# chengstone/cchess-zero

Hardware: AMD Instinct MI355X
Metric: MCTS simulations/sec (whole node), playout=1600, 7-block net (higher is better)
Workload: dtype mx6

## Files before the change

### cchess_zero_amd/csrc/cz_trunk_mx.h

```cpp
#pragma once
#include "cz_conv_kernel.h"

namespace czconv {

#include "cz_trunk_mx_asm.inc"

struct MXGeo {
    static constexpr int P = 2;
    static constexpr int ROWS = P * 90;
    static constexpr int THREADS = 512;
    static constexpr int ENT = 224;
    static constexpr int XPLANE = ENT * 16, YPLANE = ENT * 8, SPLANE = ENT * 4;
    static constexpr int X_OFF = 0, Y_OFF = 8 * XPLANE, S_OFF = Y_OFF + 8 * YPLANE;
    static constexpr int HI_OFF = S_OFF + 2 * SPLANE;
    static constexpr int ZERO_OFF = HI_OFF + ROWS * CV_ROWB;
    static constexpr int W_OFF = ZERO_OFF + CV_ROWB;
    static constexpr int SLAB_BYTES = 16384;
    static constexpr int SLAB_SHIFT = 14;
    static constexpr int SLABS_PER_LAYER = 36;
    static constexpr int LDS_BYTES = W_OFF + TW_NBUF * SLAB_BYTES;
    static constexpr int PLANES_OFF = W_OFF + 3 * SLAB_BYTES;
    static constexpr int HEADW_OFF = LDS_BYTES;
    static constexpr int LDS_TOTAL = LDS_BYTES + 3 * 128 * 4;
    static constexpr int F32_ROWB = 512;
};
static_assert(MXGeo::HI_OFF % 256 == 0 && MXGeo::W_OFF % 16 == 0, "hi rows are swizzled by their absolute 256-byte row");
static_assert(MXGeo::Y_OFF == 28672 && MXGeo::S_OFF == 43008, "tools/gen_tower_asm.py: MX_Y_OFF / MX_S_OFF");
static_assert(MXGeo::ROWS * MXGeo::F32_ROWB <= MXGeo::HEADW_OFF, "fp32 trunk rows must leave the head weights alone");
constexpr int MX_P = MXGeo::P, MX_THREADS = MXGeo::THREADS, MX_LDS_BYTES = MXGeo::LDS_TOTAL;

typedef unsigned u32x6 __attribute__((ext_vector_type(6)));
typedef _Float16 f16x8 __attribute__((ext_vector_type(8)));

__device__ __forceinline__ u32x6 mx_cvt6(f32x16 a, f32x16 b, float scale) {
    u32x6 r;
    asm volatile("v_cvt_scalef32_2xpk16_fp6_f32 %0, %1, %2, %3" : "=&v"(r) : "v"(a), "v"(b), "v"(scale));
    return r;
}

__global__ __launch_bounds__(512, 2) void k_trunk_mx_c128(const unsigned char *__restrict__ wpk,
                                                           const float *__restrict__ bias,
                                                           float *__restrict__ out,
                                                           const float *__restrict__ head_w,
                                                           const float *__restrict__ head_b,
                                                           float *__restrict__ head_out,
                                                           const uint16_t *__restrict__ planes,
                                                           const uint16_t *__restrict__ w0,
                                                           const float *__restrict__ b0,
                                                           int B, int nlayers,
                                                           const int *__restrict__ bcount,
                                                           unsigned long long *__restrict__ clk) {
    extern __shared__ __attribute__((aligned(16))) unsigned char smem[];
    using Geo = MXGeo;
    const int tid = threadIdx.x, lane = tid & 63, wave = tid >> 6;
    const int wr = wave >> 2, ct = wave & 3;
    const int l31 = lane & 31, khalf = lane >> 5;
    const int pos0 = blockIdx.x * Geo::P;
    if (bcount) {
        const int live = *bcount;
        B = live < B ? live : B;
    }
    if (pos0 >= B) return;
    unsigned long long clk_c0 = 0, clk_r0 = 0;
    if (clk) { clk_c0 = __builtin_readcyclecounter(); clk_r0 = __builtin_amdgcn_s_memrealtime(); }
    const int npos = (B - pos0) < Geo::P ? (B - pos0) : Geo::P;
    const int nrows = npos * 90;
    const int nslabs = nlayers * Geo::SLABS_PER_LAYER;
    auto lds_addr = [](int row_byte_off, int c) { return row_byte_off + ((c ^ ((row_byte_off >> 8) & 15)) << 4); };
    const unsigned voff0 = (unsigned)tid << 4, voff1 = voff0 + (unsigned)Geo::THREADS * 16u;
    const int wave_u = __builtin_amdgcn_readfirstlane(wave);
    auto lds_row_of = [](int natural) {
        const int p = natural / 90, c = natural - p * 90, y = c / 10, x = c - y * 10;
        return 20 * y + 10 * p + x;
    };

    trunk_ring_prologue<Geo>(smem, wpk, nslabs, wave_u, voff0, voff1);
    trunk_stage_planes<Geo>(smem, planes, pos0, nrows, tid);
    if (tid < 16) *reinterpret_cast<uint4 *>(smem + Geo::ZERO_OFF + (tid << 4)) = make_uint4(0, 0, 0, 0);
    if (tid < 256) *reinterpret_cast<uint4 *>(smem + Geo::X_OFF + (tid >> 5) * Geo::XPLANE + (192 + (tid & 31)) * 16) = make_uint4(0, 0, 0, 0);
    else *reinterpret_cast<uint2 *>(smem + Geo::Y_OFF + ((tid - 256) >> 5) * Geo::YPLANE + (192 + (tid & 31)) * 8) = make_uint2(0, 0);
    if (tid < 64) *reinterpret_cast<uint32_t *>(smem + Geo::S_OFF + (tid >> 5) * Geo::SPLANE + (192 + (tid & 31)) * 4) = 0x7f7f7f7fu;
    if (head_out && tid < 3 * 128 / 4)
        reinterpret_cast<float4 *>(smem + Geo::HEADW_OFF)[tid] = reinterpret_cast<const float4 *>(head_w)[tid];
    bf16x8 wf[9][2];
#pragma unroll
    for (int t = 0; t < 9; ++t)
#pragma unroll
        for (int part = 0; part < 2; ++part)
            wf[t][part] = *reinterpret_cast<const bf16x8 *>(w0 + ((size_t)(((t * 2 + part) * 2 + khalf) * 128 + ct * 32 + l31) << 3));
    asm volatile("s_waitcnt vmcnt(0)" ::: "memory");
    __syncthreads();

    int rowk[3], tapmask[3], natb[3];
#pragma unroll
    for (int i = 0; i < 3; ++i) {
        const int k = 32 * (wr * 3 + i) + l31 - 12;
        const int kk = k < 0 ? 0 : k;
        const int h = kk / 20, rem = kk - h * 20, pp = rem / 10, w = rem - pp * 10;
        rowk[i] = k;
        natb[i] = (pp * 90 + h * 10 + w) * 32;
        int m = 0;
        for (int t = 0; t < 9; ++t) {
            const int y = h + t / 3 - 1, x = w + t % 3 - 1;
            if (k >= 0 && y >= 0 && y < 9 && x >= 0 && x < 10) m |= 1 << t;
        }
        tapmask[i] = m;
    }
    auto tap_addr = [&](int tap, int (&ab)[3], int (&key)[3], int (&xr)[3], int (&yr)[3]) {
        const int delta = (tap / 3 - 1) * 20 + (tap - (tap / 3) * 3 - 1);
#pragma unroll
        for (int i = 0; i < 3; ++i) {
            const int kk = rowk[i] + delta;
            const bool on = (tapmask[i] >> tap) & 1;
            const int rb = Geo::HI_OFF + kk * CV_ROWB;
            ab[i] = on ? rb : Geo::ZERO_OFF;
            key[i] = ((rb >> 8) & 15) ^ khalf;
            xr[i] = khalf * Geo::XPLANE + ((on ? kk : 192 + (kk & 31)) << 4);
            yr[i] = xr[i] >> 1;
        }
    };
    const int vb0 = Geo::W_OFF + khalf * 2048 + ((ct * 32 + l31) << 4);
    const int vy0 = Geo::W_OFF + 12288 + khalf * 1024 + ((ct * 32 + l31) << 3);
    const int vs0 = Geo::W_OFF + 14336 + khalf * 512 + ((ct * 32 + l31) << 2);
    int keep;

    int rkk[3];
    auto refresh_rk = [&]() {
#pragma unroll
        for (int i = 0; i < 3; ++i) {
            rkk[i] = rowk[i] < 0 ? 0 : rowk[i];
            asm volatile("" : "+v"(rkk[i]));
        }
    };
    f32x16 xreg[3];
    float4 bqn[4];
    auto load_bias = [&](const float *bl) {
        int t = threadIdx.x;
        asm volatile("" : "+v"(t));
        const int boff = ((t >> 6) & 3) * 32 + 4 * ((t & 63) >> 5);
#pragma unroll
        for (int q = 0; q < 4; ++q) bqn[q] = *reinterpret_cast<const float4 *>(bl + boff + 8 * q);
    };
    auto init_acc = [&](f32x16 (&acc)[3], const float *bl, bool add_x) {
#pragma unroll
        for (int q = 0; q < 4; ++q) {
            const float4 bq = bl ? *reinterpret_cast<const float4 *>(bl + ct * 32 + 8 * q + 4 * khalf) : bqn[q];
#pragma unroll
            for (int i = 0; i < 3; ++i) {
                acc[i][4 * q + 0] = bq.x + (add_x ? xreg[i][4 * q + 0] : 0.0f);
                acc[i][4 * q + 1] = bq.y + (add_x ? xreg[i][4 * q + 1] : 0.0f);
                acc[i][4 * q + 2] = bq.z + (add_x ? xreg[i][4 * q + 2] : 0.0f);
                acc[i][4 * q + 3] = bq.w + (add_x ? xreg[i][4 * q + 3] : 0.0f);
            }
        }
    };
    auto store_tile = [&](f32x16 a, int i, bool keep_x) {
        f32x16 v;
#pragma unroll
        for (int r = 0; r < 16; ++r) v[r] = __builtin_amdgcn_fmed3f(a[r], 0.0f, 65504.0f);
        if (keep_x) xreg[i] = v;
        uint32_t pk[8];
        f32x16 hi, lo;
#pragma unroll
        for (int r = 0; r < 16; r += 2) {
            pk[r >> 1] = pack_pair<true>(f32x2{v[r], v[r + 1]});
            const f32x2 u = unpack_pair<true>(pk[r >> 1]);
            hi[r] = u[0]; hi[r + 1] = u[1];
            lo[r] = (v[r] - u[0]) * 2048.0f; lo[r + 1] = (v[r + 1] - u[1]) * 2048.0f;
        }
        float m = v[0];
#pragma unroll
        for (int r = 1; r < 16; ++r) m = fmaxf(m, v[r]);
        int byte = (int)(__float_as_uint(m) >> 23) - 2;
        byte = byte < 1 ? 1 : byte;
        const u32x6 blk = mx_cvt6(hi, lo, __uint_as_float((uint32_t)byte << 23));
        const bool live = rowk[i] >= 0;
        if (live) {
            const int rowb = Geo::HI_OFF + rkk[i] * CV_ROWB;
#pragma unroll
            for (int q = 0; q < 4; ++q) {
                const int n0 = ct * 32 + 8 * q + 4 * khalf;
                *reinterpret_cast<uint2 *>(smem + lds_addr(rowb, n0 >> 3) + ((n0 & 4) << 1)) = make_uint2(pk[2 * q], pk[2 * q + 1]);
            }
            const int g = 2 * ct + khalf;
            *reinterpret_cast<uint4 *>(smem + Geo::X_OFF + g * Geo::XPLANE + (rkk[i] << 4)) = make_uint4(blk[0], blk[1], blk[2], blk[3]);
            *reinterpret_cast<uint2 *>(smem + Geo::Y_OFF + g * Geo::YPLANE + (rkk[i] << 3)) = make_uint2(blk[4], blk[5]);
            smem[Geo::S_OFF + khalf * Geo::SPLANE + (rkk[i] << 2) + ct] = (unsigned char)byte;
        }
    };
    auto store_tile_f32 = [&](f32x16 a, int i) {
        if (rowk[i] < 0) return;
#pragma unroll
        for (int q = 0; q < 4; ++q) {
            const int c = 8 * ct + 2 * q + khalf;
            *reinterpret_cast<float4 *>(smem + rkk[i] * Geo::F32_ROWB + ((c ^ (rkk[i] & 31)) << 4)) =
                make_float4(fmaxf(a[4 * q + 0], 0.0f), fmaxf(a[4 * q + 1], 0.0f), fmaxf(a[4 * q + 2], 0.0f), fmaxf(a[4 * q + 3], 0.0f));
        }
    };

    {
        f32x16 acc[3];
        init_acc(acc, b0, false);
        load_bias(bias);
#pragma unroll
        for (int t = 0; t < 9; ++t) {
            const int shift = (t / 3 - 1) * 10 + (t % 3 - 1);
            bf16x8 af[3];
#pragma unroll
            for (int i = 0; i < 3; ++i) {
                const int a = ((tapmask[i] >> t) & 1) ? Geo::PLANES_OFF + (natb[i] + shift * 32) : Geo::ZERO_OFF;
                af[i] = *reinterpret_cast<const bf16x8 *>(smem + a + khalf * 16);
            }
#pragma unroll
            for (int part = 0; part < 2; ++part)
#pragma unroll
                for (int i = 0; i < 3; ++i)
                    acc[i] = mfma_32x32x16<true>(wf[t][part], af[i], acc[i]);
        }
        refresh_rk();
#pragma unroll
        for (int i = 0; i < 3; ++i) store_tile(acc[i], i, true);
        __syncthreads();
    }

#define MX_OPERANDS(NAB, NKEY)                                                                                       \
            : [c0] "+v"(acc[0]), [c1] "+v"(acc[1]), [c2] "+v"(acc[2]),                                                 \
              [a0h0] "+v"(fa.a[0]), [a0h1] "+v"(fa.a[1]), [a0h2] "+v"(fa.a[2]), [w0] "+v"(fa.w),                      \
              [a1h0] "+v"(fb.a[0]), [a1h1] "+v"(fb.a[1]), [a1h2] "+v"(fb.a[2]), [w1] "+v"(fb.w),                      \
              [sb0] "+v"(sb[0]), [sb1] "+v"(sb[1]), [sb2] "+v"(sb[2]),                                                \
              [t0] "=&v"(t0), [t1] "=&v"(t1), [t2] "=&v"(t2), [ws] "=&v"(wsr), [keep] "=&s"(keep)                      \
            : [ab0] "v"(ab[0]), [ab1] "v"(ab[1]), [ab2] "v"(ab[2]), [key0] "v"(key[0]), [key1] "v"(key[1]),            \
              [key2] "v"(key[2]), [nab0] "v"(NAB[0]), [nab1] "v"(NAB[1]), [nab2] "v"(NAB[2]), [nkey0] "v"(NKEY[0]),     \
              [nkey1] "v"(NKEY[1]), [nkey2] "v"(NKEY[2]), [xr0] "v"(xr[0]), [xr1] "v"(xr[1]), [xr2] "v"(xr[2]),        \
              [yr0] "v"(yr[0]), [yr1] "v"(yr[1]), [yr2] "v"(yr[2]), [vb] "v"(vb), [vy] "v"(vy), [vs] "v"(vs),          \
              [vbn] "v"(vbn), [voff0] "v"(voff0), [voff1] "v"(voff1), [sbase] "s"(sbase), [ldst] "s"(ldst)
#define MX_CLOBBERS "memory", "scc", "v232", "v233", "v234", "v235", "v236", "v237", "v238", "v239", "v240", "v241", "v242", "v243", \
                    "v244", "v245", "v246", "v247", "v248", "v249", "v250", "v251", "v252", "v253", "v254", "v255"
#define MX_ARGS()                                                                                                    \
            TRUNK_SLAB_ARGS(wpk, const int vy = vy0 + slot; const int vs = vs0 + slot;)
#define MX_RUN(ASMSTR, NAB, NKEY)                                                                                    \
        {                                                                                                            \
            MX_ARGS()                                                                                                \
            asm volatile(ASMSTR MX_OPERANDS(NAB, NKEY) : MX_CLOBBERS);                                               \
            ++g;                                                                                                     \
        }
#define MX_RUNV(ASMSTR, NAB, NKEY)                           \
        {                                                                                                            \
            MX_ARGS()                                                                                                \
            asm volatile(ASMSTR MX_OPERANDS(NAB, NKEY), [skipm] "s"(skipm) : MX_CLOBBERS, "vcc");                    \
            ++g;                                                                                                     \
        }

#ifdef MX_TIMING
    unsigned long long tm_loop = 0, tm_epi = 0, tm_set = 0, tm_t0 = __builtin_readcyclecounter();
    const unsigned long long tm_first = tm_t0 - clk_c0;
#define MX_TM(acc) { const unsigned long long n_ = __builtin_readcyclecounter(); acc += n_ - tm_t0; tm_t0 = n_; }
#else
#define MX_TM(acc)
#endif
    struct MxFrag { bf16x8 a[3], w; };
    int g = 0;
    int skipm;
    asm volatile("s_cmp_lt_u32 %1, 4\n\ts_cselect_b32 %0, 1, 0" : "=s"(skipm) : "s"(wave_u) : "scc");
#pragma unroll 1
    for (int layer = 0; layer < nlayers; ++layer) {
        f32x16 acc[3];
        init_acc(acc, nullptr, (layer & 1) != 0);
        int ab[3], key[3], nab[3], nkey[3], xr[3], yr[3], nxr[3], nyr[3], t0, t1, t2, wsr;
        int sb[3] = {0, 0, 0};
        MxFrag fa, fb;
        tap_addr(0, ab, key, xr, yr);
        {
            const int vb = vb0 + (((unsigned)g & 3u) << Geo::SLAB_SHIFT);
#pragma unroll
            for (int i = 0; i < 3; ++i) {
                fa.a[i] = *reinterpret_cast<const bf16x8 *>(smem + ab[i] + ((0 ^ key[i]) << 4));
                fb.a[i] = *reinterpret_cast<const bf16x8 *>(smem + ab[i] + ((2 ^ key[i]) << 4));
            }
            fa.w = *reinterpret_cast<const bf16x8 *>(smem + vb);
            fb.w = *reinterpret_cast<const bf16x8 *>(smem + vb + 4096);
            asm volatile("" : "+v"(fa.a[0]), "+v"(fa.a[1]), "+v"(fa.a[2]), "+v"(fa.w), "+v"(fb.a[0]), "+v"(fb.a[1]), "+v"(fb.a[2]), "+v"(fb.w));
        }
        MX_TM(tm_set)
        int tap = 0;
#pragma unroll 1
        for (; tap < 3; ++tap) {
            MX_RUNV(MX_SKIP0_ASM_Q0, ab, key)
            MX_RUNV(MX_SKIP0_ASM_Q1, ab, key)
            MX_RUNV(MX_SKIP0_ASM_Q2, ab, key)
            tap_addr(tap + 1, nab, nkey, nxr, nyr);
            MX_RUNV(MX_SKIP0_ASM_Q3, nab, nkey)
#pragma unroll
            for (int i = 0; i < 3; ++i) { ab[i] = nab[i]; key[i] = nkey[i]; xr[i] = nxr[i]; yr[i] = nyr[i]; }
        }
#pragma unroll 1
        for (; tap < 8; ++tap) {
            MX_RUN(MX_SLAB_ASM_Q0, ab, key)
            MX_RUN(MX_SLAB_ASM_Q1, ab, key)
            MX_RUN(MX_SLAB_ASM_Q2, ab, key)
            tap_addr(tap + 1, nab, nkey, nxr, nyr);
            MX_RUN(MX_SLAB_ASM_Q3, nab, nkey)
#pragma unroll
            for (int i = 0; i < 3; ++i) { ab[i] = nab[i]; key[i] = nkey[i]; xr[i] = nxr[i]; yr[i] = nyr[i]; }
        }
        MX_RUN(MX_SLAB_ASM_Q0, ab, key)
        MX_RUN(MX_SLAB_ASM_Q1, ab, key)
        MX_RUN(MX_SLAB_ASM_Q2, ab, key)
        MX_RUN(MX_SLAB_ASM_Q3_LAST, ab, key)
        const bool last = layer + 1 == nlayers;
        if (last) asm volatile("s_waitcnt vmcnt(0)" ::: "memory");
        else load_bias(bias + (layer + 1) * 128);
        asm volatile("s_nop 15\n\ts_nop 15\n\ts_nop 15" ::: "memory");
        MX_TM(tm_loop)
        refresh_rk();
        if (last) {
#pragma unroll
            for (int i = 0; i < 3; ++i) store_tile_f32(acc[i], i);
        } else {
#pragma unroll
            for (int i = 0; i < 3; ++i) store_tile(acc[i], i, (layer & 1) != 0);
        }
        __syncthreads();
        MX_TM(tm_epi)
    }
    if (clk && tid == 0) {
        clk[blockIdx.x * 4 + 0] = clk_c0; clk[blockIdx.x * 4 + 1] = __builtin_readcyclecounter();
        clk[blockIdx.x * 4 + 2] = clk_r0; clk[blockIdx.x * 4 + 3] = __builtin_amdgcn_s_memrealtime();
#ifdef MX_TIMING
        clk[blockIdx.x * 4 + 0] = tm_first; clk[blockIdx.x * 4 + 1] = tm_loop; clk[blockIdx.x * 4 + 2] = tm_epi; clk[blockIdx.x * 4 + 3] = tm_set;
#endif
    }
    asm volatile("s_waitcnt vmcnt(0)" ::: "memory");
    if (out) {
        float4 *go = reinterpret_cast<float4 *>(out + (size_t)pos0 * 90 * 128);
        for (int idx = tid; idx < nrows * 32; idx += Geo::THREADS) {
            const int r = idx >> 5, c = idx & 31, k = lds_row_of(r);
            go[idx] = *reinterpret_cast<const float4 *>(smem + k * Geo::F32_ROWB + ((c ^ (k & 31)) << 4));
        }
    }
    if (head_out) {
        const float *hw = reinterpret_cast<const float *>(smem + Geo::HEADW_OFF);
        for (int r = tid; r < nrows; r += Geo::THREADS) {
            const int k = lds_row_of(r);
            float acc0 = 0.f, acc1 = 0.f, acc2 = 0.f;
#pragma unroll 4
            for (int c = 0; c < 32; ++c) {
                const float4 e = *reinterpret_cast<const float4 *>(smem + k * Geo::F32_ROWB + ((c ^ (k & 31)) << 4));
                const float *w0_ = hw + c * 4, *w1_ = hw + 128 + c * 4, *w2_ = hw + 256 + c * 4;
                acc0 += e.x * w0_[0] + e.y * w0_[1] + e.z * w0_[2] + e.w * w0_[3];
                acc1 += e.x * w1_[0] + e.y * w1_[1] + e.z * w1_[2] + e.w * w1_[3];
                acc2 += e.x * w2_[0] + e.y * w2_[1] + e.z * w2_[2] + e.w * w2_[3];
            }
            float *o = head_out + ((size_t)pos0 * 90 + r) * 3;
            o[0] = fmaxf(acc0 + head_b[0], 0.f);
            o[1] = fmaxf(acc1 + head_b[1], 0.f);
            o[2] = fmaxf(acc2 + head_b[2], 0.f);
        }
    }
}
#undef MX_OPERANDS
#undef MX_CLOBBERS
#undef MX_ARGS
#undef MX_RUN
#undef MX_RUNV

}
```

### cchess_zero_amd/csrc/cz_trunk_mx_asm.inc

```
#define MX_SLAB_ASM_Q0 \
    "s_mov_b32 %[keep], m0\n\t" \
    "s_waitcnt lgkmcnt(4)\n\t" \
    "v_mfma_f32_32x32x16_f16 %[c0], %[w0], %[a0h0], %[c0]\n\t" \
    "ds_read_b128 v[232:235], %[xr0] offset:0\n\t" \
    "ds_read_b64 v[236:237], %[yr0] offset:28672\n\t" \
    "ds_read_b128 v[238:241], %[xr1] offset:0\n\t" \
    "ds_read_b64 v[242:243], %[yr1] offset:28672\n\t" \
    "v_lshrrev_b32 %[t0], 1, %[yr0]\n\t" \
    "v_lshrrev_b32 %[t1], 1, %[yr1]\n\t" \
    "v_lshrrev_b32 %[t2], 1, %[yr2]\n\t" \
    "v_mfma_f32_32x32x16_f16 %[c1], %[w0], %[a0h1], %[c1]\n\t" \
    "ds_read_b128 v[244:247], %[xr2] offset:0\n\t" \
    "ds_read_b64 v[248:249], %[yr2] offset:28672\n\t" \
    "ds_read_b32 %[sb0], %[t0] offset:43008\n\t" \
    "ds_read_b32 %[sb1], %[t1] offset:43008\n\t" \
    "ds_read_b32 %[sb2], %[t2] offset:43008\n\t" \
    "v_mfma_f32_32x32x16_f16 %[c2], %[w0], %[a0h2], %[c2]\n\t" \
    "ds_read_b128 v[250:253], %[vb] offset:8192\n\t" \
    "ds_read_b64 v[254:255], %[vy]\n\t" \
    "ds_read_b32 %[ws], %[vs]\n\t" \
    "s_waitcnt vmcnt(2)\n\t" \
    "s_barrier\n\t" \
    "s_waitcnt lgkmcnt(12)\n\t" \
    "v_mfma_f32_32x32x16_f16 %[c0], %[w1], %[a1h0], %[c0]\n\t" \
    "v_xor_b32 %[t0], 4, %[key0]\n\t" \
    "v_xor_b32 %[t1], 4, %[key1]\n\t" \
    "v_xor_b32 %[t2], 4, %[key2]\n\t" \
    "v_lshl_add_u32 %[t0], %[t0], 4, %[ab0]\n\t" \
    "v_lshl_add_u32 %[t1], %[t1], 4, %[ab1]\n\t" \
    "v_lshl_add_u32 %[t2], %[t2], 4, %[ab2]\n\t" \
    "v_mfma_f32_32x32x16_f16 %[c1], %[w1], %[a1h1], %[c1]\n\t" \
    "ds_read_b128 %[a0h0], %[t0]\n\t" \
    "ds_read_b128 %[a0h1], %[t1]\n\t" \
    "v_mfma_f32_32x32x16_f16 %[c2], %[w1], %[a1h2], %[c2]\n\t" \
    "ds_read_b128 %[a0h2], %[t2]\n\t" \
    "ds_read_b128 %[w0], %[vbn]\n\t" \
    "s_waitcnt lgkmcnt(4)\n\t" \
    "v_mfma_scale_f32_32x32x64_f8f6f4 %[c0], v[250:255], v[232:237], %[c0], %[ws], %[sb0] op_sel:[0,0,0] op_sel_hi:[0,0,0] cbsz:2 blgp:2\n\t" \
    "v_xor_b32 %[t0], 6, %[key0]\n\t" \
    "v_xor_b32 %[t1], 6, %[key1]\n\t" \
    "v_xor_b32 %[t2], 6, %[key2]\n\t" \
    "v_lshl_add_u32 %[t0], %[t0], 4, %[ab0]\n\t" \
    "v_lshl_add_u32 %[t1], %[t1], 4, %[ab1]\n\t" \
    "v_lshl_add_u32 %[t2], %[t2], 4, %[ab2]\n\t" \
    "s_mov_b32 m0, %[ldst]\n\t" \
    "s_nop 0\n\t" \
    "global_load_lds_dwordx4 %[voff0], %[sbase]\n\t" \
    "v_mfma_scale_f32_32x32x64_f8f6f4 %[c1], v[250:255], v[238:243], %[c1], %[ws], %[sb1] op_sel:[0,0,0] op_sel_hi:[0,0,0] cbsz:2 blgp:2\n\t" \
    "ds_read_b128 %[a1h0], %[t0]\n\t" \
    "ds_read_b128 %[a1h1], %[t1]\n\t" \
    "s_add_u32 m0, %[ldst], 0x2000\n\t" \
    "s_nop 0\n\t" \
    "global_load_lds_dwordx4 %[voff1], %[sbase]\n\t" \
    "v_mfma_scale_f32_32x32x64_f8f6f4 %[c2], v[250:255], v[244:249], %[c2], %[ws], %[sb2] op_sel:[0,0,0] op_sel_hi:[0,0,0] cbsz:2 blgp:2\n\t" \
    "ds_read_b128 %[a1h2], %[t2]\n\t" \
    "ds_read_b128 %[w1], %[vbn] offset:4096\n\t" \
    "s_mov_b32 m0, %[keep]\n\t"

#define MX_SLAB_ASM_Q1 \
    "s_mov_b32 %[keep], m0\n\t" \
    "s_waitcnt lgkmcnt(4)\n\t" \
    "v_mfma_f32_32x32x16_f16 %[c0], %[w0], %[a0h0], %[c0]\n\t" \
    "ds_read_b128 v[232:235], %[xr0] offset:7168\n\t" \
    "ds_read_b64 v[236:237], %[yr0] offset:32256\n\t" \
    "ds_read_b128 v[238:241], %[xr1] offset:7168\n\t" \
    "ds_read_b64 v[242:243], %[yr1] offset:32256\n\t" \
    "v_mfma_f32_32x32x16_f16 %[c1], %[w0], %[a0h1], %[c1]\n\t" \
    "ds_read_b128 v[244:247], %[xr2] offset:7168\n\t" \
    "ds_read_b64 v[248:249], %[yr2] offset:32256\n\t" \
    "v_mfma_f32_32x32x16_f16 %[c2], %[w0], %[a0h2], %[c2]\n\t" \
    "ds_read_b128 v[250:253], %[vb] offset:8192\n\t" \
    "ds_read_b64 v[254:255], %[vy]\n\t" \
    "ds_read_b32 %[ws], %[vs]\n\t" \
    "s_waitcnt vmcnt(2)\n\t" \
    "s_barrier\n\t" \
    "s_waitcnt lgkmcnt(9)\n\t" \
    "v_mfma_f32_32x32x16_f16 %[c0], %[w1], %[a1h0], %[c0]\n\t" \
    "v_xor_b32 %[t0], 8, %[key0]\n\t" \
    "v_xor_b32 %[t1], 8, %[key1]\n\t" \
    "v_xor_b32 %[t2], 8, %[key2]\n\t" \
    "v_lshl_add_u32 %[t0], %[t0], 4, %[ab0]\n\t" \
    "v_lshl_add_u32 %[t1], %[t1], 4, %[ab1]\n\t" \
    "v_lshl_add_u32 %[t2], %[t2], 4, %[ab2]\n\t" \
    "v_mfma_f32_32x32x16_f16 %[c1], %[w1], %[a1h1], %[c1]\n\t" \
    "ds_read_b128 %[a0h0], %[t0]\n\t" \
    "ds_read_b128 %[a0h1], %[t1]\n\t" \
    "v_mfma_f32_32x32x16_f16 %[c2], %[w1], %[a1h2], %[c2]\n\t" \
    "ds_read_b128 %[a0h2], %[t2]\n\t" \
    "ds_read_b128 %[w0], %[vbn]\n\t" \
    "s_waitcnt lgkmcnt(4)\n\t" \
    "v_mfma_scale_f32_32x32x64_f8f6f4 %[c0], v[250:255], v[232:237], %[c0], %[ws], %[sb0] op_sel:[0,1,0] op_sel_hi:[0,0,0] cbsz:2 blgp:2\n\t" \
    "v_xor_b32 %[t0], 10, %[key0]\n\t" \
    "v_xor_b32 %[t1], 10, %[key1]\n\t" \
    "v_xor_b32 %[t2], 10, %[key2]\n\t" \
    "v_lshl_add_u32 %[t0], %[t0], 4, %[ab0]\n\t" \
    "v_lshl_add_u32 %[t1], %[t1], 4, %[ab1]\n\t" \
    "v_lshl_add_u32 %[t2], %[t2], 4, %[ab2]\n\t" \
    "s_mov_b32 m0, %[ldst]\n\t" \
    "s_nop 0\n\t" \
    "global_load_lds_dwordx4 %[voff0], %[sbase]\n\t" \
    "v_mfma_scale_f32_32x32x64_f8f6f4 %[c1], v[250:255], v[238:243], %[c1], %[ws], %[sb1] op_sel:[0,1,0] op_sel_hi:[0,0,0] cbsz:2 blgp:2\n\t" \
    "ds_read_b128 %[a1h0], %[t0]\n\t" \
    "ds_read_b128 %[a1h1], %[t1]\n\t" \
    "s_add_u32 m0, %[ldst], 0x2000\n\t" \
    "s_nop 0\n\t" \
    "global_load_lds_dwordx4 %[voff1], %[sbase]\n\t" \
    "v_mfma_scale_f32_32x32x64_f8f6f4 %[c2], v[250:255], v[244:249], %[c2], %[ws], %[sb2] op_sel:[0,1,0] op_sel_hi:[0,0,0] cbsz:2 blgp:2\n\t" \
    "ds_read_b128 %[a1h2], %[t2]\n\t" \
    "ds_read_b128 %[w1], %[vbn] offset:4096\n\t" \
    "s_mov_b32 m0, %[keep]\n\t"

#define MX_SLAB_ASM_Q2 \
    "s_mov_b32 %[keep], m0\n\t" \
    "s_waitcnt lgkmcnt(4)\n\t" \
    "v_mfma_f32_32x32x16_f16 %[c0], %[w0], %[a0h0], %[c0]\n\t" \
    "ds_read_b128 v[232:235], %[xr0] offset:14336\n\t" \
    "ds_read_b64 v[236:237], %[yr0] offset:35840\n\t" \
    "ds_read_b128 v[238:241], %[xr1] offset:14336\n\t" \
    "ds_read_b64 v[242:243], %[yr1] offset:35840\n\t" \
    "v_mfma_f32_32x32x16_f16 %[c1], %[w0], %[a0h1], %[c1]\n\t" \
    "ds_read_b128 v[244:247], %[xr2] offset:14336\n\t" \
    "ds_read_b64 v[248:249], %[yr2] offset:35840\n\t" \
    "v_mfma_f32_32x32x16_f16 %[c2], %[w0], %[a0h2], %[c2]\n\t" \
    "ds_read_b128 v[250:253], %[vb] offset:8192\n\t" \
    "ds_read_b64 v[254:255], %[vy]\n\t" \
    "ds_read_b32 %[ws], %[vs]\n\t" \
    "s_waitcnt vmcnt(2)\n\t" \
    "s_barrier\n\t" \
    "s_waitcnt lgkmcnt(9)\n\t" \
    "v_mfma_f32_32x32x16_f16 %[c0], %[w1], %[a1h0], %[c0]\n\t" \
    "v_xor_b32 %[t0], 12, %[key0]\n\t" \
    "v_xor_b32 %[t1], 12, %[key1]\n\t" \
    "v_xor_b32 %[t2], 12, %[key2]\n\t" \
    "v_lshl_add_u32 %[t0], %[t0], 4, %[ab0]\n\t" \
    "v_lshl_add_u32 %[t1], %[t1], 4, %[ab1]\n\t" \
    "v_lshl_add_u32 %[t2], %[t2], 4, %[ab2]\n\t" \
    "v_mfma_f32_32x32x16_f16 %[c1], %[w1], %[a1h1], %[c1]\n\t" \
    "ds_read_b128 %[a0h0], %[t0]\n\t" \
    "ds_read_b128 %[a0h1], %[t1]\n\t" \
    "v_mfma_f32_32x32x16_f16 %[c2], %[w1], %[a1h2], %[c2]\n\t" \
    "ds_read_b128 %[a0h2], %[t2]\n\t" \
    "ds_read_b128 %[w0], %[vbn]\n\t" \
    "s_waitcnt lgkmcnt(4)\n\t" \
    "v_mfma_scale_f32_32x32x64_f8f6f4 %[c0], v[250:255], v[232:237], %[c0], %[ws], %[sb0] op_sel:[0,0,0] op_sel_hi:[0,1,0] cbsz:2 blgp:2\n\t" \
    "v_xor_b32 %[t0], 14, %[key0]\n\t" \
    "v_xor_b32 %[t1], 14, %[key1]\n\t" \
    "v_xor_b32 %[t2], 14, %[key2]\n\t" \
    "v_lshl_add_u32 %[t0], %[t0], 4, %[ab0]\n\t" \
    "v_lshl_add_u32 %[t1], %[t1], 4, %[ab1]\n\t" \
    "v_lshl_add_u32 %[t2], %[t2], 4, %[ab2]\n\t" \
    "s_mov_b32 m0, %[ldst]\n\t" \
    "s_nop 0\n\t" \
    "global_load_lds_dwordx4 %[voff0], %[sbase]\n\t" \
    "v_mfma_scale_f32_32x32x64_f8f6f4 %[c1], v[250:255], v[238:243], %[c1], %[ws], %[sb1] op_sel:[0,0,0] op_sel_hi:[0,1,0] cbsz:2 blgp:2\n\t" \
    "ds_read_b128 %[a1h0], %[t0]\n\t" \
    "ds_read_b128 %[a1h1], %[t1]\n\t" \
    "s_add_u32 m0, %[ldst], 0x2000\n\t" \
    "s_nop 0\n\t" \
    "global_load_lds_dwordx4 %[voff1], %[sbase]\n\t" \
    "v_mfma_scale_f32_32x32x64_f8f6f4 %[c2], v[250:255], v[244:249], %[c2], %[ws], %[sb2] op_sel:[0,0,0] op_sel_hi:[0,1,0] cbsz:2 blgp:2\n\t" \
    "ds_read_b128 %[a1h2], %[t2]\n\t" \
    "ds_read_b128 %[w1], %[vbn] offset:4096\n\t" \
    "s_mov_b32 m0, %[keep]\n\t"

#define MX_SLAB_ASM_Q3 \
    "s_mov_b32 %[keep], m0\n\t" \
    "s_waitcnt lgkmcnt(4)\n\t" \
    "v_mfma_f32_32x32x16_f16 %[c0], %[w0], %[a0h0], %[c0]\n\t" \
    "ds_read_b128 v[232:235], %[xr0] offset:21504\n\t" \
    "ds_read_b64 v[236:237], %[yr0] offset:39424\n\t" \
    "ds_read_b128 v[238:241], %[xr1] offset:21504\n\t" \
    "ds_read_b64 v[242:243], %[yr1] offset:39424\n\t" \
    "v_mfma_f32_32x32x16_f16 %[c1], %[w0], %[a0h1], %[c1]\n\t" \
    "ds_read_b128 v[244:247], %[xr2] offset:21504\n\t" \
    "ds_read_b64 v[248:249], %[yr2] offset:39424\n\t" \
    "v_mfma_f32_32x32x16_f16 %[c2], %[w0], %[a0h2], %[c2]\n\t" \
    "ds_read_b128 v[250:253], %[vb] offset:8192\n\t" \
    "ds_read_b64 v[254:255], %[vy]\n\t" \
    "ds_read_b32 %[ws], %[vs]\n\t" \
    "s_waitcnt vmcnt(2)\n\t" \
    "s_barrier\n\t" \
    "s_waitcnt lgkmcnt(9)\n\t" \
    "v_mfma_f32_32x32x16_f16 %[c0], %[w1], %[a1h0], %[c0]\n\t" \
    "v_xor_b32 %[t0], 0, %[nkey0]\n\t" \
    "v_xor_b32 %[t1], 0, %[nkey1]\n\t" \
    "v_xor_b32 %[t2], 0, %[nkey2]\n\t" \
    "v_lshl_add_u32 %[t0], %[t0], 4, %[nab0]\n\t" \
    "v_lshl_add_u32 %[t1], %[t1], 4, %[nab1]\n\t" \
    "v_lshl_add_u32 %[t2], %[t2], 4, %[nab2]\n\t" \
    "v_mfma_f32_32x32x16_f16 %[c1], %[w1], %[a1h1], %[c1]\n\t" \
    "ds_read_b128 %[a0h0], %[t0]\n\t" \
    "ds_read_b128 %[a0h1], %[t1]\n\t" \
    "v_mfma_f32_32x32x16_f16 %[c2], %[w1], %[a1h2], %[c2]\n\t" \
    "ds_read_b128 %[a0h2], %[t2]\n\t" \
    "ds_read_b128 %[w0], %[vbn]\n\t" \
    "s_waitcnt lgkmcnt(4)\n\t" \
    "v_mfma_scale_f32_32x32x64_f8f6f4 %[c0], v[250:255], v[232:237], %[c0], %[ws], %[sb0] op_sel:[0,1,0] op_sel_hi:[0,1,0] cbsz:2 blgp:2\n\t" \
    "v_xor_b32 %[t0], 2, %[nkey0]\n\t" \
    "v_xor_b32 %[t1], 2, %[nkey1]\n\t" \
    "v_xor_b32 %[t2], 2, %[nkey2]\n\t" \
    "v_lshl_add_u32 %[t0], %[t0], 4, %[nab0]\n\t" \
    "v_lshl_add_u32 %[t1], %[t1], 4, %[nab1]\n\t" \
    "v_lshl_add_u32 %[t2], %[t2], 4, %[nab2]\n\t" \
    "s_mov_b32 m0, %[ldst]\n\t" \
    "s_nop 0\n\t" \
    "global_load_lds_dwordx4 %[voff0], %[sbase]\n\t" \
    "v_mfma_scale_f32_32x32x64_f8f6f4 %[c1], v[250:255], v[238:243], %[c1], %[ws], %[sb1] op_sel:[0,1,0] op_sel_hi:[0,1,0] cbsz:2 blgp:2\n\t" \
    "ds_read_b128 %[a1h0], %[t0]\n\t" \
    "ds_read_b128 %[a1h1], %[t1]\n\t" \
    "s_add_u32 m0, %[ldst], 0x2000\n\t" \
    "s_nop 0\n\t" \
    "global_load_lds_dwordx4 %[voff1], %[sbase]\n\t" \
    "v_mfma_scale_f32_32x32x64_f8f6f4 %[c2], v[250:255], v[244:249], %[c2], %[ws], %[sb2] op_sel:[0,1,0] op_sel_hi:[0,1,0] cbsz:2 blgp:2\n\t" \
    "ds_read_b128 %[a1h2], %[t2]\n\t" \
    "ds_read_b128 %[w1], %[vbn] offset:4096\n\t" \
    "s_mov_b32 m0, %[keep]\n\t"

#define MX_SKIP0_ASM_Q0 \
    "s_cmp_lg_u32 %[skipm], 0\n\t" \
    "s_cselect_b64 vcc, -1, 0\n\t" \
    "s_mov_b32 %[keep], m0\n\t" \
    "s_waitcnt lgkmcnt(4)\n\t" \
    "s_cbranch_vccnz 1f\n\t" \
    "v_mfma_f32_32x32x16_f16 %[c0], %[w0], %[a0h0], %[c0]\n\t" \
    "1:\n\t" \
    "ds_read_b128 v[232:235], %[xr0] offset:0\n\t" \
    "ds_read_b64 v[236:237], %[yr0] offset:28672\n\t" \
    "ds_read_b128 v[238:241], %[xr1] offset:0\n\t" \
    "ds_read_b64 v[242:243], %[yr1] offset:28672\n\t" \
    "v_lshrrev_b32 %[t0], 1, %[yr0]\n\t" \
    "v_lshrrev_b32 %[t1], 1, %[yr1]\n\t" \
    "v_lshrrev_b32 %[t2], 1, %[yr2]\n\t" \
    "v_mfma_f32_32x32x16_f16 %[c1], %[w0], %[a0h1], %[c1]\n\t" \
    "ds_read_b128 v[244:247], %[xr2] offset:0\n\t" \
    "ds_read_b64 v[248:249], %[yr2] offset:28672\n\t" \
    "ds_read_b32 %[sb0], %[t0] offset:43008\n\t" \
    "ds_read_b32 %[sb1], %[t1] offset:43008\n\t" \
    "ds_read_b32 %[sb2], %[t2] offset:43008\n\t" \
    "v_mfma_f32_32x32x16_f16 %[c2], %[w0], %[a0h2], %[c2]\n\t" \
    "ds_read_b128 v[250:253], %[vb] offset:8192\n\t" \
    "ds_read_b64 v[254:255], %[vy]\n\t" \
    "ds_read_b32 %[ws], %[vs]\n\t" \
    "s_waitcnt vmcnt(2)\n\t" \
    "s_barrier\n\t" \
    "s_waitcnt lgkmcnt(12)\n\t" \
    "s_cbranch_vccnz 1f\n\t" \
    "v_mfma_f32_32x32x16_f16 %[c0], %[w1], %[a1h0], %[c0]\n\t" \
    "1:\n\t" \
    "v_xor_b32 %[t0], 4, %[key0]\n\t" \
    "v_xor_b32 %[t1], 4, %[key1]\n\t" \
    "v_xor_b32 %[t2], 4, %[key2]\n\t" \
    "v_lshl_add_u32 %[t0], %[t0], 4, %[ab0]\n\t" \
    "v_lshl_add_u32 %[t1], %[t1], 4, %[ab1]\n\t" \
    "v_lshl_add_u32 %[t2], %[t2], 4, %[ab2]\n\t" \
    "v_mfma_f32_32x32x16_f16 %[c1], %[w1], %[a1h1], %[c1]\n\t" \
    "ds_read_b128 %[a0h0], %[t0]\n\t" \
    "ds_read_b128 %[a0h1], %[t1]\n\t" \
    "v_mfma_f32_32x32x16_f16 %[c2], %[w1], %[a1h2], %[c2]\n\t" \
    "ds_read_b128 %[a0h2], %[t2]\n\t" \
    "ds_read_b128 %[w0], %[vbn]\n\t" \
    "s_waitcnt lgkmcnt(4)\n\t" \
    "s_cbranch_vccnz 1f\n\t" \
    "v_mfma_scale_f32_32x32x64_f8f6f4 %[c0], v[250:255], v[232:237], %[c0], %[ws], %[sb0] op_sel:[0,0,0] op_sel_hi:[0,0,0] cbsz:2 blgp:2\n\t" \
    "1:\n\t" \
    "v_xor_b32 %[t0], 6, %[key0]\n\t" \
    "v_xor_b32 %[t1], 6, %[key1]\n\t" \
    "v_xor_b32 %[t2], 6, %[key2]\n\t" \
    "v_lshl_add_u32 %[t0], %[t0], 4, %[ab0]\n\t" \
    "v_lshl_add_u32 %[t1], %[t1], 4, %[ab1]\n\t" \
    "v_lshl_add_u32 %[t2], %[t2], 4, %[ab2]\n\t" \
    "s_mov_b32 m0, %[ldst]\n\t" \
    "s_nop 0\n\t" \
    "global_load_lds_dwordx4 %[voff0], %[sbase]\n\t" \
    "v_mfma_scale_f32_32x32x64_f8f6f4 %[c1], v[250:255], v[238:243], %[c1], %[ws], %[sb1] op_sel:[0,0,0] op_sel_hi:[0,0,0] cbsz:2 blgp:2\n\t" \
    "ds_read_b128 %[a1h0], %[t0]\n\t" \
    "ds_read_b128 %[a1h1], %[t1]\n\t" \
    "s_add_u32 m0, %[ldst], 0x2000\n\t" \
    "s_nop 0\n\t" \
    "global_load_lds_dwordx4 %[voff1], %[sbase]\n\t" \
    "v_mfma_scale_f32_32x32x64_f8f6f4 %[c2], v[250:255], v[244:249], %[c2], %[ws], %[sb2] op_sel:[0,0,0] op_sel_hi:[0,0,0] cbsz:2 blgp:2\n\t" \
    "ds_read_b128 %[a1h2], %[t2]\n\t" \
    "ds_read_b128 %[w1], %[vbn] offset:4096\n\t" \
    "s_mov_b32 m0, %[keep]\n\t"

#define MX_SKIP0_ASM_Q1 \
    "s_cmp_lg_u32 %[skipm], 0\n\t" \
    "s_cselect_b64 vcc, -1, 0\n\t" \
    "s_mov_b32 %[keep], m0\n\t" \
    "s_waitcnt lgkmcnt(4)\n\t" \
    "s_cbranch_vccnz 1f\n\t" \
    "v_mfma_f32_32x32x16_f16 %[c0], %[w0], %[a0h0], %[c0]\n\t" \
    "1:\n\t" \
    "ds_read_b128 v[232:235], %[xr0] offset:7168\n\t" \
    "ds_read_b64 v[236:237], %[yr0] offset:32256\n\t" \
    "ds_read_b128 v[238:241], %[xr1] offset:7168\n\t" \
    "ds_read_b64 v[242:243], %[yr1] offset:32256\n\t" \
    "v_mfma_f32_32x32x16_f16 %[c1], %[w0], %[a0h1], %[c1]\n\t" \
    "ds_read_b128 v[244:247], %[xr2] offset:7168\n\t" \
    "ds_read_b64 v[248:249], %[yr2] offset:32256\n\t" \
    "v_mfma_f32_32x32x16_f16 %[c2], %[w0], %[a0h2], %[c2]\n\t" \
    "ds_read_b128 v[250:253], %[vb] offset:8192\n\t" \
    "ds_read_b64 v[254:255], %[vy]\n\t" \
    "ds_read_b32 %[ws], %[vs]\n\t" \
    "s_waitcnt vmcnt(2)\n\t" \
    "s_barrier\n\t" \
    "s_waitcnt lgkmcnt(9)\n\t" \
    "s_cbranch_vccnz 1f\n\t" \
    "v_mfma_f32_32x32x16_f16 %[c0], %[w1], %[a1h0], %[c0]\n\t" \
    "1:\n\t" \
    "v_xor_b32 %[t0], 8, %[key0]\n\t" \
    "v_xor_b32 %[t1], 8, %[key1]\n\t" \
    "v_xor_b32 %[t2], 8, %[key2]\n\t" \
    "v_lshl_add_u32 %[t0], %[t0], 4, %[ab0]\n\t" \
    "v_lshl_add_u32 %[t1], %[t1], 4, %[ab1]\n\t" \
    "v_lshl_add_u32 %[t2], %[t2], 4, %[ab2]\n\t" \
    "v_mfma_f32_32x32x16_f16 %[c1], %[w1], %[a1h1], %[c1]\n\t" \
    "ds_read_b128 %[a0h0], %[t0]\n\t" \
    "ds_read_b128 %[a0h1], %[t1]\n\t" \
    "v_mfma_f32_32x32x16_f16 %[c2], %[w1], %[a1h2], %[c2]\n\t" \
    "ds_read_b128 %[a0h2], %[t2]\n\t" \
    "ds_read_b128 %[w0], %[vbn]\n\t" \
    "s_waitcnt lgkmcnt(4)\n\t" \
    "s_cbranch_vccnz 1f\n\t" \
    "v_mfma_scale_f32_32x32x64_f8f6f4 %[c0], v[250:255], v[232:237], %[c0], %[ws], %[sb0] op_sel:[0,1,0] op_sel_hi:[0,0,0] cbsz:2 blgp:2\n\t" \
    "1:\n\t" \
    "v_xor_b32 %[t0], 10, %[key0]\n\t" \
    "v_xor_b32 %[t1], 10, %[key1]\n\t" \
    "v_xor_b32 %[t2], 10, %[key2]\n\t" \
    "v_lshl_add_u32 %[t0], %[t0], 4, %[ab0]\n\t" \
    "v_lshl_add_u32 %[t1], %[t1], 4, %[ab1]\n\t" \
    "v_lshl_add_u32 %[t2], %[t2], 4, %[ab2]\n\t" \
    "s_mov_b32 m0, %[ldst]\n\t" \
    "s_nop 0\n\t" \
    "global_load_lds_dwordx4 %[voff0], %[sbase]\n\t" \
    "v_mfma_scale_f32_32x32x64_f8f6f4 %[c1], v[250:255], v[238:243], %[c1], %[ws], %[sb1] op_sel:[0,1,0] op_sel_hi:[0,0,0] cbsz:2 blgp:2\n\t" \
    "ds_read_b128 %[a1h0], %[t0]\n\t" \
    "ds_read_b128 %[a1h1], %[t1]\n\t" \
    "s_add_u32 m0, %[ldst], 0x2000\n\t" \
    "s_nop 0\n\t" \
    "global_load_lds_dwordx4 %[voff1], %[sbase]\n\t" \
    "v_mfma_scale_f32_32x32x64_f8f6f4 %[c2], v[250:255], v[244:249], %[c2], %[ws], %[sb2] op_sel:[0,1,0] op_sel_hi:[0,0,0] cbsz:2 blgp:2\n\t" \
    "ds_read_b128 %[a1h2], %[t2]\n\t" \
    "ds_read_b128 %[w1], %[vbn] offset:4096\n\t" \
    "s_mov_b32 m0, %[keep]\n\t"

#define MX_SKIP0_ASM_Q2 \
    "s_cmp_lg_u32 %[skipm], 0\n\t" \
    "s_cselect_b64 vcc, -1, 0\n\t" \
    "s_mov_b32 %[keep], m0\n\t" \
    "s_waitcnt lgkmcnt(4)\n\t" \
    "s_cbranch_vccnz 1f\n\t" \
    "v_mfma_f32_32x32x16_f16 %[c0], %[w0], %[a0h0], %[c0]\n\t" \
    "1:\n\t" \
    "ds_read_b128 v[232:235], %[xr0] offset:14336\n\t" \
    "ds_read_b64 v[236:237], %[yr0] offset:35840\n\t" \
    "ds_read_b128 v[238:241], %[xr1] offset:14336\n\t" \
    "ds_read_b64 v[242:243], %[yr1] offset:35840\n\t" \
    "v_mfma_f32_32x32x16_f16 %[c1], %[w0], %[a0h1], %[c1]\n\t" \
    "ds_read_b128 v[244:247], %[xr2] offset:14336\n\t" \
    "ds_read_b64 v[248:249], %[yr2] offset:35840\n\t" \
    "v_mfma_f32_32x32x16_f16 %[c2], %[w0], %[a0h2], %[c2]\n\t" \
    "ds_read_b128 v[250:253], %[vb] offset:8192\n\t" \
    "ds_read_b64 v[254:255], %[vy]\n\t" \
    "ds_read_b32 %[ws], %[vs]\n\t" \
    "s_waitcnt vmcnt(2)\n\t" \
    "s_barrier\n\t" \
    "s_waitcnt lgkmcnt(9)\n\t" \
    "s_cbranch_vccnz 1f\n\t" \
    "v_mfma_f32_32x32x16_f16 %[c0], %[w1], %[a1h0], %[c0]\n\t" \
    "1:\n\t" \
    "v_xor_b32 %[t0], 12, %[key0]\n\t" \
    "v_xor_b32 %[t1], 12, %[key1]\n\t" \
    "v_xor_b32 %[t2], 12, %[key2]\n\t" \
    "v_lshl_add_u32 %[t0], %[t0], 4, %[ab0]\n\t" \
    "v_lshl_add_u32 %[t1], %[t1], 4, %[ab1]\n\t" \
    "v_lshl_add_u32 %[t2], %[t2], 4, %[ab2]\n\t" \
    "v_mfma_f32_32x32x16_f16 %[c1], %[w1], %[a1h1], %[c1]\n\t" \
    "ds_read_b128 %[a0h0], %[t0]\n\t" \
    "ds_read_b128 %[a0h1], %[t1]\n\t" \
    "v_mfma_f32_32x32x16_f16 %[c2], %[w1], %[a1h2], %[c2]\n\t" \
    "ds_read_b128 %[a0h2], %[t2]\n\t" \
    "ds_read_b128 %[w0], %[vbn]\n\t" \
    "s_waitcnt lgkmcnt(4)\n\t" \
    "s_cbranch_vccnz 1f\n\t" \
    "v_mfma_scale_f32_32x32x64_f8f6f4 %[c0], v[250:255], v[232:237], %[c0], %[ws], %[sb0] op_sel:[0,0,0] op_sel_hi:[0,1,0] cbsz:2 blgp:2\n\t" \
    "1:\n\t" \
    "v_xor_b32 %[t0], 14, %[key0]\n\t" \
    "v_xor_b32 %[t1], 14, %[key1]\n\t" \
    "v_xor_b32 %[t2], 14, %[key2]\n\t" \
    "v_lshl_add_u32 %[t0], %[t0], 4, %[ab0]\n\t" \
    "v_lshl_add_u32 %[t1], %[t1], 4, %[ab1]\n\t" \
    "v_lshl_add_u32 %[t2], %[t2], 4, %[ab2]\n\t" \
    "s_mov_b32 m0, %[ldst]\n\t" \
    "s_nop 0\n\t" \
    "global_load_lds_dwordx4 %[voff0], %[sbase]\n\t" \
    "v_mfma_scale_f32_32x32x64_f8f6f4 %[c1], v[250:255], v[238:243], %[c1], %[ws], %[sb1] op_sel:[0,0,0] op_sel_hi:[0,1,0] cbsz:2 blgp:2\n\t" \
    "ds_read_b128 %[a1h0], %[t0]\n\t" \
    "ds_read_b128 %[a1h1], %[t1]\n\t" \
    "s_add_u32 m0, %[ldst], 0x2000\n\t" \
    "s_nop 0\n\t" \
    "global_load_lds_dwordx4 %[voff1], %[sbase]\n\t" \
    "v_mfma_scale_f32_32x32x64_f8f6f4 %[c2], v[250:255], v[244:249], %[c2], %[ws], %[sb2] op_sel:[0,0,0] op_sel_hi:[0,1,0] cbsz:2 blgp:2\n\t" \
    "ds_read_b128 %[a1h2], %[t2]\n\t" \
    "ds_read_b128 %[w1], %[vbn] offset:4096\n\t" \
    "s_mov_b32 m0, %[keep]\n\t"

#define MX_SKIP0_ASM_Q3 \
    "s_cmp_lg_u32 %[skipm], 0\n\t" \
    "s_cselect_b64 vcc, -1, 0\n\t" \
    "s_mov_b32 %[keep], m0\n\t" \
    "s_waitcnt lgkmcnt(4)\n\t" \
    "s_cbranch_vccnz 1f\n\t" \
    "v_mfma_f32_32x32x16_f16 %[c0], %[w0], %[a0h0], %[c0]\n\t" \
    "1:\n\t" \
    "ds_read_b128 v[232:235], %[xr0] offset:21504\n\t" \
    "ds_read_b64 v[236:237], %[yr0] offset:39424\n\t" \
    "ds_read_b128 v[238:241], %[xr1] offset:21504\n\t" \
    "ds_read_b64 v[242:243], %[yr1] offset:39424\n\t" \
    "v_mfma_f32_32x32x16_f16 %[c1], %[w0], %[a0h1], %[c1]\n\t" \
    "ds_read_b128 v[244:247], %[xr2] offset:21504\n\t" \
    "ds_read_b64 v[248:249], %[yr2] offset:39424\n\t" \
    "v_mfma_f32_32x32x16_f16 %[c2], %[w0], %[a0h2], %[c2]\n\t" \
    "ds_read_b128 v[250:253], %[vb] offset:8192\n\t" \
    "ds_read_b64 v[254:255], %[vy]\n\t" \
    "ds_read_b32 %[ws], %[vs]\n\t" \
    "s_waitcnt vmcnt(2)\n\t" \
    "s_barrier\n\t" \
    "s_waitcnt lgkmcnt(9)\n\t" \
    "s_cbranch_vccnz 1f\n\t" \
    "v_mfma_f32_32x32x16_f16 %[c0], %[w1], %[a1h0], %[c0]\n\t" \
    "1:\n\t" \
    "v_xor_b32 %[t0], 0, %[nkey0]\n\t" \
    "v_xor_b32 %[t1], 0, %[nkey1]\n\t" \
    "v_xor_b32 %[t2], 0, %[nkey2]\n\t" \
    "v_lshl_add_u32 %[t0], %[t0], 4, %[nab0]\n\t" \
    "v_lshl_add_u32 %[t1], %[t1], 4, %[nab1]\n\t" \
    "v_lshl_add_u32 %[t2], %[t2], 4, %[nab2]\n\t" \
    "v_mfma_f32_32x32x16_f16 %[c1], %[w1], %[a1h1], %[c1]\n\t" \
    "ds_read_b128 %[a0h0], %[t0]\n\t" \
    "ds_read_b128 %[a0h1], %[t1]\n\t" \
    "v_mfma_f32_32x32x16_f16 %[c2], %[w1], %[a1h2], %[c2]\n\t" \
    "ds_read_b128 %[a0h2], %[t2]\n\t" \
    "ds_read_b128 %[w0], %[vbn]\n\t" \
    "s_waitcnt lgkmcnt(4)\n\t" \
    "s_cbranch_vccnz 1f\n\t" \
    "v_mfma_scale_f32_32x32x64_f8f6f4 %[c0], v[250:255], v[232:237], %[c0], %[ws], %[sb0] op_sel:[0,1,0] op_sel_hi:[0,1,0] cbsz:2 blgp:2\n\t" \
    "1:\n\t" \
    "v_xor_b32 %[t0], 2, %[nkey0]\n\t" \
    "v_xor_b32 %[t1], 2, %[nkey1]\n\t" \
    "v_xor_b32 %[t2], 2, %[nkey2]\n\t" \
    "v_lshl_add_u32 %[t0], %[t0], 4, %[nab0]\n\t" \
    "v_lshl_add_u32 %[t1], %[t1], 4, %[nab1]\n\t" \
    "v_lshl_add_u32 %[t2], %[t2], 4, %[nab2]\n\t" \
    "s_mov_b32 m0, %[ldst]\n\t" \
    "s_nop 0\n\t" \
    "global_load_lds_dwordx4 %[voff0], %[sbase]\n\t" \
    "v_mfma_scale_f32_32x32x64_f8f6f4 %[c1], v[250:255], v[238:243], %[c1], %[ws], %[sb1] op_sel:[0,1,0] op_sel_hi:[0,1,0] cbsz:2 blgp:2\n\t" \
    "ds_read_b128 %[a1h0], %[t0]\n\t" \
    "ds_read_b128 %[a1h1], %[t1]\n\t" \
    "s_add_u32 m0, %[ldst], 0x2000\n\t" \
    "s_nop 0\n\t" \
    "global_load_lds_dwordx4 %[voff1], %[sbase]\n\t" \
    "v_mfma_scale_f32_32x32x64_f8f6f4 %[c2], v[250:255], v[244:249], %[c2], %[ws], %[sb2] op_sel:[0,1,0] op_sel_hi:[0,1,0] cbsz:2 blgp:2\n\t" \
    "ds_read_b128 %[a1h2], %[t2]\n\t" \
    "ds_read_b128 %[w1], %[vbn] offset:4096\n\t" \
    "s_mov_b32 m0, %[keep]\n\t"

#define MX_SLAB_ASM_Q3_LAST \
    "s_mov_b32 %[keep], m0\n\t" \
    "s_waitcnt lgkmcnt(4)\n\t" \
    "v_mfma_f32_32x32x16_f16 %[c0], %[w0], %[a0h0], %[c0]\n\t" \
    "ds_read_b128 v[232:235], %[xr0] offset:21504\n\t" \
    "ds_read_b64 v[236:237], %[yr0] offset:39424\n\t" \
    "ds_read_b128 v[238:241], %[xr1] offset:21504\n\t" \
    "ds_read_b64 v[242:243], %[yr1] offset:39424\n\t" \
    "v_mfma_f32_32x32x16_f16 %[c1], %[w0], %[a0h1], %[c1]\n\t" \
    "ds_read_b128 v[244:247], %[xr2] offset:21504\n\t" \
    "ds_read_b64 v[248:249], %[yr2] offset:39424\n\t" \
    "v_mfma_f32_32x32x16_f16 %[c2], %[w0], %[a0h2], %[c2]\n\t" \
    "ds_read_b128 v[250:253], %[vb] offset:8192\n\t" \
    "ds_read_b64 v[254:255], %[vy]\n\t" \
    "ds_read_b32 %[ws], %[vs]\n\t" \
    "s_waitcnt vmcnt(2) lgkmcnt(0)\n\t" \
    "s_barrier\n\t" \
    "v_mfma_f32_32x32x16_f16 %[c0], %[w1], %[a1h0], %[c0]\n\t" \
    "v_mfma_f32_32x32x16_f16 %[c1], %[w1], %[a1h1], %[c1]\n\t" \
    "v_mfma_f32_32x32x16_f16 %[c2], %[w1], %[a1h2], %[c2]\n\t" \
    "v_mfma_scale_f32_32x32x64_f8f6f4 %[c0], v[250:255], v[232:237], %[c0], %[ws], %[sb0] op_sel:[0,1,0] op_sel_hi:[0,1,0] cbsz:2 blgp:2\n\t" \
    "s_mov_b32 m0, %[ldst]\n\t" \
    "s_nop 0\n\t" \
    "global_load_lds_dwordx4 %[voff0], %[sbase]\n\t" \
    "v_mfma_scale_f32_32x32x64_f8f6f4 %[c1], v[250:255], v[238:243], %[c1], %[ws], %[sb1] op_sel:[0,1,0] op_sel_hi:[0,1,0] cbsz:2 blgp:2\n\t" \
    "s_add_u32 m0, %[ldst], 0x2000\n\t" \
    "s_nop 0\n\t" \
    "global_load_lds_dwordx4 %[voff1], %[sbase]\n\t" \
    "v_mfma_scale_f32_32x32x64_f8f6f4 %[c2], v[250:255], v[244:249], %[c2], %[ws], %[sb2] op_sel:[0,1,0] op_sel_hi:[0,1,0] cbsz:2 blgp:2\n\t" \
    "s_mov_b32 m0, %[keep]\n\t"
```

Before: 1.977 million.

## Bake weight-ring slot offsets into slab asm immediates and raise producer wave priority

Each quarter-slab asm body now addresses its fixed ring slot (g & 3) through immediate ds_read offsets and m0 adds from constant per-thread bases. This replaces the per-slab vb/vy/vs/vbn/ldst recomputation in TRUNK_SLAB_ARGS and should cut VALU/SALU address math and register pressure in the hot loop. It relies on SLABS_PER_LAYER being a multiple of 4 so slab index and ring slot stay aligned, which a new static_assert checks. Waves 0-3 also get raised scheduling priority via s_setprio.

Measured after the change: 1.997 million, median of 6. 1.01x the previous value.

```diff
diff --git a/cchess_zero_amd/csrc/cz_trunk_mx.h b/cchess_zero_amd/csrc/cz_trunk_mx.h
--- a/cchess_zero_amd/csrc/cz_trunk_mx.h
+++ b/cchess_zero_amd/csrc/cz_trunk_mx.h
@@ -26,6 +26,8 @@
 };
 static_assert(MXGeo::HI_OFF % 256 == 0 && MXGeo::W_OFF % 16 == 0, "hi rows are swizzled by their absolute 256-byte row");
 static_assert(MXGeo::Y_OFF == 28672 && MXGeo::S_OFF == 43008, "tools/gen_tower_asm.py: MX_Y_OFF / MX_S_OFF");
+static_assert(MXGeo::SLABS_PER_LAYER % 4 == 0 && MXGeo::SLAB_BYTES == 16384 && 3 * MXGeo::SLAB_BYTES + 14336 < 65536,
+              "tools/gen_tower_asm.py: slab g of a layer sits in ring slot g & 3 = its quarter, an immediate of the slab bodies (MX_SLAB)");
 static_assert(MXGeo::ROWS * MXGeo::F32_ROWB <= MXGeo::HEADW_OFF, "fp32 trunk rows must leave the head weights alone");
 constexpr int MX_P = MXGeo::P, MX_THREADS = MXGeo::THREADS, MX_LDS_BYTES = MXGeo::LDS_TOTAL;
 
@@ -122,6 +124,7 @@
     const int vb0 = Geo::W_OFF + khalf * 2048 + ((ct * 32 + l31) << 4);
     const int vy0 = Geo::W_OFF + 12288 + khalf * 1024 + ((ct * 32 + l31) << 3);
     const int vs0 = Geo::W_OFF + 14336 + khalf * 512 + ((ct * 32 + l31) << 2);
+    const int ldst0 = Geo::W_OFF + (wave_u << 10);
     int keep;
 
     int rkk[3];
@@ -232,12 +235,13 @@
             : [ab0] "v"(ab[0]), [ab1] "v"(ab[1]), [ab2] "v"(ab[2]), [key0] "v"(key[0]), [key1] "v"(key[1]),            \
               [key2] "v"(key[2]), [nab0] "v"(NAB[0]), [nab1] "v"(NAB[1]), [nab2] "v"(NAB[2]), [nkey0] "v"(NKEY[0]),     \
               [nkey1] "v"(NKEY[1]), [nkey2] "v"(NKEY[2]), [xr0] "v"(xr[0]), [xr1] "v"(xr[1]), [xr2] "v"(xr[2]),        \
-              [yr0] "v"(yr[0]), [yr1] "v"(yr[1]), [yr2] "v"(yr[2]), [vb] "v"(vb), [vy] "v"(vy), [vs] "v"(vs),          \
-              [vbn] "v"(vbn), [voff0] "v"(voff0), [voff1] "v"(voff1), [sbase] "s"(sbase), [ldst] "s"(ldst)
+              [yr0] "v"(yr[0]), [yr1] "v"(yr[1]), [yr2] "v"(yr[2]), [vb] "v"(vb0), [vy] "v"(vy0), [vs] "v"(vs0),       \
+              [voff0] "v"(voff0), [voff1] "v"(voff1), [sbase] "s"(sbase), [ldst] "s"(ldst0)
 #define MX_CLOBBERS "memory", "scc", "v232", "v233", "v234", "v235", "v236", "v237", "v238", "v239", "v240", "v241", "v242", "v243", \
                     "v244", "v245", "v246", "v247", "v248", "v249", "v250", "v251", "v252", "v253", "v254", "v255"
-#define MX_ARGS()                                                                                                    \
-            TRUNK_SLAB_ARGS(wpk, const int vy = vy0 + slot; const int vs = vs0 + slot;)
+#define MX_ARGS()    \
+            const int gn = g + 3 < nslabs ? g + 3 : nslabs - 1;    \
+            const unsigned char *sbase = wpk + (size_t)gn * Geo::SLAB_BYTES;
 #define MX_RUN(ASMSTR, NAB, NKEY)                                                                                    \
         {                                                                                                            \
             MX_ARGS()                                                                                                \
@@ -262,6 +266,7 @@
     int g = 0;
     int skipm;
     asm volatile("s_cmp_lt_u32 %1, 4\n\ts_cselect_b32 %0, 1, 0" : "=s"(skipm) : "s"(wave_u) : "scc");
+    if (wave_u < 4) __builtin_amdgcn_s_setprio(1);
 #pragma unroll 1
     for (int layer = 0; layer < nlayers; ++layer) {
         f32x16 acc[3];
@@ -271,7 +276,7 @@
         MxFrag fa, fb;
         tap_addr(0, ab, key, xr, yr);
         {
-            const int vb = vb0 + (((unsigned)g & 3u) << Geo::SLAB_SHIFT);
+            const int vb = vb0;
 #pragma unroll
             for (int i = 0; i < 3; ++i) {
                 fa.a[i] = *reinterpret_cast<const bf16x8 *>(smem + ab[i] + ((0 ^ key[i]) << 4));
diff --git a/cchess_zero_amd/csrc/cz_trunk_mx_asm.inc b/cchess_zero_amd/csrc/cz_trunk_mx_asm.inc
--- a/cchess_zero_amd/csrc/cz_trunk_mx_asm.inc
+++ b/cchess_zero_amd/csrc/cz_trunk_mx_asm.inc
@@ -17,8 +17,8 @@
     "ds_read_b32 %[sb2], %[t2] offset:43008\n\t" \
     "v_mfma_f32_32x32x16_f16 %[c2], %[w0], %[a0h2], %[c2]\n\t" \
     "ds_read_b128 v[250:253], %[vb] offset:8192\n\t" \
-    "ds_read_b64 v[254:255], %[vy]\n\t" \
-    "ds_read_b32 %[ws], %[vs]\n\t" \
+    "ds_read_b64 v[254:255], %[vy] offset:0\n\t" \
+    "ds_read_b32 %[ws], %[vs] offset:0\n\t" \
     "s_waitcnt vmcnt(2)\n\t" \
     "s_barrier\n\t" \
     "s_waitcnt lgkmcnt(12)\n\t" \
@@ -34,7 +34,7 @@
     "ds_read_b128 %[a0h1], %[t1]\n\t" \
     "v_mfma_f32_32x32x16_f16 %[c2], %[w1], %[a1h2], %[c2]\n\t" \
     "ds_read_b128 %[a0h2], %[t2]\n\t" \
-    "ds_read_b128 %[w0], %[vbn]\n\t" \
+    "ds_read_b128 %[w0], %[vb] offset:16384\n\t" \
     "s_waitcnt lgkmcnt(4)\n\t" \
     "v_mfma_scale_f32_32x32x64_f8f6f4 %[c0], v[250:255], v[232:237], %[c0], %[ws], %[sb0] op_sel:[0,0,0] op_sel_hi:[0,0,0] cbsz:2 blgp:2\n\t" \
     "v_xor_b32 %[t0], 6, %[key0]\n\t" \
@@ -43,18 +43,18 @@
     "v_lshl_add_u32 %[t0], %[t0], 4, %[ab0]\n\t" \
     "v_lshl_add_u32 %[t1], %[t1], 4, %[ab1]\n\t" \
     "v_lshl_add_u32 %[t2], %[t2], 4, %[ab2]\n\t" \
-    "s_mov_b32 m0, %[ldst]\n\t" \
+    "s_add_u32 m0, %[ldst], 0xc000\n\t" \
     "s_nop 0\n\t" \
     "global_load_lds_dwordx4 %[voff0], %[sbase]\n\t" \
     "v_mfma_scale_f32_32x32x64_f8f6f4 %[c1], v[250:255], v[238:243], %[c1], %[ws], %[sb1] op_sel:[0,0,0] op_sel_hi:[0,0,0] cbsz:2 blgp:2\n\t" \
     "ds_read_b128 %[a1h0], %[t0]\n\t" \
     "ds_read_b128 %[a1h1], %[t1]\n\t" \
-    "s_add_u32 m0, %[ldst], 0x2000\n\t" \
+    "s_add_u32 m0, %[ldst], 0xe000\n\t" \
     "s_nop 0\n\t" \
     "global_load_lds_dwordx4 %[voff1], %[sbase]\n\t" \
     "v_mfma_scale_f32_32x32x64_f8f6f4 %[c2], v[250:255], v[244:249], %[c2], %[ws], %[sb2] op_sel:[0,0,0] op_sel_hi:[0,0,0] cbsz:2 blgp:2\n\t" \
     "ds_read_b128 %[a1h2], %[t2]\n\t" \
-    "ds_read_b128 %[w1], %[vbn] offset:4096\n\t" \
+    "ds_read_b128 %[w1], %[vb] offset:20480\n\t" \
     "s_mov_b32 m0, %[keep]\n\t"
 
 #define MX_SLAB_ASM_Q1 \
@@ -69,9 +69,9 @@
     "ds_read_b128 v[244:247], %[xr2] offset:7168\n\t" \
     "ds_read_b64 v[248:249], %[yr2] offset:32256\n\t" \
     "v_mfma_f32_32x32x16_f16 %[c2], %[w0], %[a0h2], %[c2]\n\t" \
-    "ds_read_b128 v[250:253], %[vb] offset:8192\n\t" \
-    "ds_read_b64 v[254:255], %[vy]\n\t" \
-    "ds_read_b32 %[ws], %[vs]\n\t" \
+    "ds_read_b128 v[250:253], %[vb] offset:24576\n\t" \
+    "ds_read_b64 v[254:255], %[vy] offset:16384\n\t" \
+    "ds_read_b32 %[ws], %[vs] offset:16384\n\t" \
     "s_waitcnt vmcnt(2)\n\t" \
     "s_barrier\n\t" \
     "s_waitcnt lgkmcnt(9)\n\t" \
@@ -87,7 +87,7 @@
     "ds_read_b128 %[a0h1], %[t1]\n\t" \
     "v_mfma_f32_32x32x16_f16 %[c2], %[w1], %[a1h2], %[c2]\n\t" \
     "ds_read_b128 %[a0h2], %[t2]\n\t" \
-    "ds_read_b128 %[w0], %[vbn]\n\t" \
+    "ds_read_b128 %[w0], %[vb] offset:32768\n\t" \
     "s_waitcnt lgkmcnt(4)\n\t" \
     "v_mfma_scale_f32_32x32x64_f8f6f4 %[c0], v[250:255], v[232:237], %[c0], %[ws], %[sb0] op_sel:[0,1,0] op_sel_hi:[0,0,0] cbsz:2 blgp:2\n\t" \
     "v_xor_b32 %[t0], 10, %[key0]\n\t" \
@@ -96,7 +96,7 @@
     "v_lshl_add_u32 %[t0], %[t0], 4, %[ab0]\n\t" \
     "v_lshl_add_u32 %[t1], %[t1], 4, %[ab1]\n\t" \
     "v_lshl_add_u32 %[t2], %[t2], 4, %[ab2]\n\t" \
-    "s_mov_b32 m0, %[ldst]\n\t" \
+    "s_add_u32 m0, %[ldst], 0x0\n\t" \
     "s_nop 0\n\t" \
     "global_load_lds_dwordx4 %[voff0], %[sbase]\n\t" \
     "v_mfma_scale_f32_32x32x64_f8f6f4 %[c1], v[250:255], v[238:243], %[c1], %[ws], %[sb1] op_sel:[0,1,0] op_sel_hi:[0,0,0] cbsz:2 blgp:2\n\t" \
@@ -107,7 +107,7 @@
     "global_load_lds_dwordx4 %[voff1], %[sbase]\n\t" \
     "v_mfma_scale_f32_32x32x64_f8f6f4 %[c2], v[250:255], v[244:249], %[c2], %[ws], %[sb2] op_sel:[0,1,0] op_sel_hi:[0,0,0] cbsz:2 blgp:2\n\t" \
     "ds_read_b128 %[a1h2], %[t2]\n\t" \
-    "ds_read_b128 %[w1], %[vbn] offset:4096\n\t" \
+    "ds_read_b128 %[w1], %[vb] offset:36864\n\t" \
     "s_mov_b32 m0, %[keep]\n\t"
 
 #define MX_SLAB_ASM_Q2 \
@@ -122,9 +122,9 @@
     "ds_read_b128 v[244:247], %[xr2] offset:14336\n\t" \
     "ds_read_b64 v[248:249], %[yr2] offset:35840\n\t" \
     "v_mfma_f32_32x32x16_f16 %[c2], %[w0], %[a0h2], %[c2]\n\t" \
-    "ds_read_b128 v[250:253], %[vb] offset:8192\n\t" \
-    "ds_read_b64 v[254:255], %[vy]\n\t" \
-    "ds_read_b32 %[ws], %[vs]\n\t" \
+    "ds_read_b128 v[250:253], %[vb] offset:40960\n\t" \
+    "ds_read_b64 v[254:255], %[vy] offset:32768\n\t" \
+    "ds_read_b32 %[ws], %[vs] offset:32768\n\t" \
     "s_waitcnt vmcnt(2)\n\t" \
     "s_barrier\n\t" \
     "s_waitcnt lgkmcnt(9)\n\t" \
@@ -140,7 +140,7 @@
     "ds_read_b128 %[a0h1], %[t1]\n\t" \
     "v_mfma_f32_32x32x16_f16 %[c2], %[w1], %[a1h2], %[c2]\n\t" \
     "ds_read_b128 %[a0h2], %[t2]\n\t" \
-    "ds_read_b128 %[w0], %[vbn]\n\t" \
+    "ds_read_b128 %[w0], %[vb] offset:49152\n\t" \
     "s_waitcnt lgkmcnt(4)\n\t" \
     "v_mfma_scale_f32_32x32x64_f8f6f4 %[c0], v[250:255], v[232:237], %[c0], %[ws], %[sb0] op_sel:[0,0,0] op_sel_hi:[0,1,0] cbsz:2 blgp:2\n\t" \
     "v_xor_b32 %[t0], 14, %[key0]\n\t" \
@@ -149,18 +149,18 @@
     "v_lshl_add_u32 %[t0], %[t0], 4, %[ab0]\n\t" \
     "v_lshl_add_u32 %[t1], %[t1], 4, %[ab1]\n\t" \
     "v_lshl_add_u32 %[t2], %[t2], 4, %[ab2]\n\t" \
-    "s_mov_b32 m0, %[ldst]\n\t" \
+    "s_add_u32 m0, %[ldst], 0x4000\n\t" \
     "s_nop 0\n\t" \
     "global_load_lds_dwordx4 %[voff0], %[sbase]\n\t" \
     "v_mfma_scale_f32_32x32x64_f8f6f4 %[c1], v[250:255], v[238:243], %[c1], %[ws], %[sb1] op_sel:[0,0,0] op_sel_hi:[0,1,0] cbsz:2 blgp:2\n\t" \
     "ds_read_b128 %[a1h0], %[t0]\n\t" \
     "ds_read_b128 %[a1h1], %[t1]\n\t" \
-    "s_add_u32 m0, %[ldst], 0x2000\n\t" \
+    "s_add_u32 m0, %[ldst], 0x6000\n\t" \
     "s_nop 0\n\t" \
     "global_load_lds_dwordx4 %[voff1], %[sbase]\n\t" \
     "v_mfma_scale_f32_32x32x64_f8f6f4 %[c2], v[250:255], v[244:249], %[c2], %[ws], %[sb2] op_sel:[0,0,0] op_sel_hi:[0,1,0] cbsz:2 blgp:2\n\t" \
     "ds_read_b128 %[a1h2], %[t2]\n\t" \
-    "ds_read_b128 %[w1], %[vbn] offset:4096\n\t" \
+    "ds_read_b128 %[w1], %[vb] offset:53248\n\t" \
     "s_mov_b32 m0, %[keep]\n\t"
 
 #define MX_SLAB_ASM_Q3 \
@@ -175,9 +175,9 @@
     "ds_read_b128 v[244:247], %[xr2] offset:21504\n\t" \
     "ds_read_b64 v[248:249], %[yr2] offset:39424\n\t" \
     "v_mfma_f32_32x32x16_f16 %[c2], %[w0], %[a0h2], %[c2]\n\t" \
-    "ds_read_b128 v[250:253], %[vb] offset:8192\n\t" \
-    "ds_read_b64 v[254:255], %[vy]\n\t" \
-    "ds_read_b32 %[ws], %[vs]\n\t" \
+    "ds_read_b128 v[250:253], %[vb] offset:57344\n\t" \
+    "ds_read_b64 v[254:255], %[vy] offset:49152\n\t" \
+    "ds_read_b32 %[ws], %[vs] offset:49152\n\t" \
     "s_waitcnt vmcnt(2)\n\t" \
     "s_barrier\n\t" \
     "s_waitcnt lgkmcnt(9)\n\t" \
@@ -193,7 +193,7 @@
     "ds_read_b128 %[a0h1], %[t1]\n\t" \
     "v_mfma_f32_32x32x16_f16 %[c2], %[w1], %[a1h2], %[c2]\n\t" \
     "ds_read_b128 %[a0h2], %[t2]\n\t" \
-    "ds_read_b128 %[w0], %[vbn]\n\t" \
+    "ds_read_b128 %[w0], %[vb] offset:0\n\t" \
     "s_waitcnt lgkmcnt(4)\n\t" \
     "v_mfma_scale_f32_32x32x64_f8f6f4 %[c0], v[250:255], v[232:237], %[c0], %[ws], %[sb0] op_sel:[0,1,0] op_sel_hi:[0,1,0] cbsz:2 blgp:2\n\t" \
     "v_xor_b32 %[t0], 2, %[nkey0]\n\t" \
@@ -202,18 +202,18 @@
     "v_lshl_add_u32 %[t0], %[t0], 4, %[nab0]\n\t" \
     "v_lshl_add_u32 %[t1], %[t1], 4, %[nab1]\n\t" \
     "v_lshl_add_u32 %[t2], %[t2], 4, %[nab2]\n\t" \
-    "s_mov_b32 m0, %[ldst]\n\t" \
+    "s_add_u32 m0, %[ldst], 0x8000\n\t" \
     "s_nop 0\n\t" \
     "global_load_lds_dwordx4 %[voff0], %[sbase]\n\t" \
     "v_mfma_scale_f32_32x32x64_f8f6f4 %[c1], v[250:255], v[238:243], %[c1], %[ws], %[sb1] op_sel:[0,1,0] op_sel_hi:[0,1,0] cbsz:2 blgp:2\n\t" \
     "ds_read_b128 %[a1h0], %[t0]\n\t" \
     "ds_read_b128 %[a1h1], %[t1]\n\t" \
-    "s_add_u32 m0, %[ldst], 0x2000\n\t" \
+    "s_add_u32 m0, %[ldst], 0xa000\n\t" \
     "s_nop 0\n\t" \
     "global_load_lds_dwordx4 %[voff1], %[sbase]\n\t" \
     "v_mfma_scale_f32_32x32x64_f8f6f4 %[c2], v[250:255], v[244:249], %[c2], %[ws], %[sb2] op_sel:[0,1,0] op_sel_hi:[0,1,0] cbsz:2 blgp:2\n\t" \
     "ds_read_b128 %[a1h2], %[t2]\n\t" \
-    "ds_read_b128 %[w1], %[vbn] offset:4096\n\t" \
+    "ds_read_b128 %[w1], %[vb] offset:4096\n\t" \
     "s_mov_b32 m0, %[keep]\n\t"
 
 #define MX_SKIP0_ASM_Q0 \
@@ -239,8 +239,8 @@
     "ds_read_b32 %[sb2], %[t2] offset:43008\n\t" \
     "v_mfma_f32_32x32x16_f16 %[c2], %[w0], %[a0h2], %[c2]\n\t" \
     "ds_read_b128 v[250:253], %[vb] offset:8192\n\t" \
-    "ds_read_b64 v[254:255], %[vy]\n\t" \
-    "ds_read_b32 %[ws], %[vs]\n\t" \
+    "ds_read_b64 v[254:255], %[vy] offset:0\n\t" \
+    "ds_read_b32 %[ws], %[vs] offset:0\n\t" \
     "s_waitcnt vmcnt(2)\n\t" \
     "s_barrier\n\t" \
     "s_waitcnt lgkmcnt(12)\n\t" \
@@ -258,7 +258,7 @@
     "ds_read_b128 %[a0h1], %[t1]\n\t" \
     "v_mfma_f32_32x32x16_f16 %[c2], %[w1], %[a1h2], %[c2]\n\t" \
     "ds_read_b128 %[a0h2], %[t2]\n\t" \
-    "ds_read_b128 %[w0], %[vbn]\n\t" \
+    "ds_read_b128 %[w0], %[vb] offset:16384\n\t" \
     "s_waitcnt lgkmcnt(4)\n\t" \
     "s_cbranch_vccnz 1f\n\t" \
     "v_mfma_scale_f32_32x32x64_f8f6f4 %[c0], v[250:255], v[232:237], %[c0], %[ws], %[sb0] op_sel:[0,0,0] op_sel_hi:[0,0,0] cbsz:2 blgp:2\n\t" \
@@ -269,18 +269,18 @@
     "v_lshl_add_u32 %[t0], %[t0], 4, %[ab0]\n\t" \
     "v_lshl_add_u32 %[t1], %[t1], 4, %[ab1]\n\t" \
     "v_lshl_add_u32 %[t2], %[t2], 4, %[ab2]\n\t" \
-    "s_mov_b32 m0, %[ldst]\n\t" \
+    "s_add_u32 m0, %[ldst], 0xc000\n\t" \
     "s_nop 0\n\t" \
     "global_load_lds_dwordx4 %[voff0], %[sbase]\n\t" \
     "v_mfma_scale_f32_32x32x64_f8f6f4 %[c1], v[250:255], v[238:243], %[c1], %[ws], %[sb1] op_sel:[0,0,0] op_sel_hi:[0,0,0] cbsz:2 blgp:2\n\t" \
     "ds_read_b128 %[a1h0], %[t0]\n\t" \
     "ds_read_b128 %[a1h1], %[t1]\n\t" \
-    "s_add_u32 m0, %[ldst], 0x2000\n\t" \
+    "s_add_u32 m0, %[ldst], 0xe000\n\t" \
     "s_nop 0\n\t" \
     "global_load_lds_dwordx4 %[voff1], %[sbase]\n\t" \
     "v_mfma_scale_f32_32x32x64_f8f6f4 %[c2], v[250:255], v[244:249], %[c2], %[ws], %[sb2] op_sel:[0,0,0] op_sel_hi:[0,0,0] cbsz:2 blgp:2\n\t" \
     "ds_read_b128 %[a1h2], %[t2]\n\t" \
-    "ds_read_b128 %[w1], %[vbn] offset:4096\n\t" \
+    "ds_read_b128 %[w1], %[vb] offset:20480\n\t" \
     "s_mov_b32 m0, %[keep]\n\t"
 
 #define MX_SKIP0_ASM_Q1 \
@@ -299,9 +299,9 @@
     "ds_read_b128 v[244:247], %[xr2] offset:7168\n\t" \
     "ds_read_b64 v[248:249], %[yr2] offset:32256\n\t" \
     "v_mfma_f32_32x32x16_f16 %[c2], %[w0], %[a0h2], %[c2]\n\t" \
-    "ds_read_b128 v[250:253], %[vb] offset:8192\n\t" \
-    "ds_read_b64 v[254:255], %[vy]\n\t" \
-    "ds_read_b32 %[ws], %[vs]\n\t" \
+    "ds_read_b128 v[250:253], %[vb] offset:24576\n\t" \
+    "ds_read_b64 v[254:255], %[vy] offset:16384\n\t" \
+    "ds_read_b32 %[ws], %[vs] offset:16384\n\t" \
     "s_waitcnt vmcnt(2)\n\t" \
     "s_barrier\n\t" \
     "s_waitcnt lgkmcnt(9)\n\t" \
@@ -319,7 +319,7 @@
     "ds_read_b128 %[a0h1], %[t1]\n\t" \
     "v_mfma_f32_32x32x16_f16 %[c2], %[w1], %[a1h2], %[c2]\n\t" \
     "ds_read_b128 %[a0h2], %[t2]\n\t" \
-    "ds_read_b128 %[w0], %[vbn]\n\t" \
+    "ds_read_b128 %[w0], %[vb] offset:32768\n\t" \
     "s_waitcnt lgkmcnt(4)\n\t" \
     "s_cbranch_vccnz 1f\n\t" \
     "v_mfma_scale_f32_32x32x64_f8f6f4 %[c0], v[250:255], v[232:237], %[c0], %[ws], %[sb0] op_sel:[0,1,0] op_sel_hi:[0,0,0] cbsz:2 blgp:2\n\t" \
@@ -330,7 +330,7 @@
     "v_lshl_add_u32 %[t0], %[t0], 4, %[ab0]\n\t" \
     "v_lshl_add_u32 %[t1], %[t1], 4, %[ab1]\n\t" \
     "v_lshl_add_u32 %[t2], %[t2], 4, %[ab2]\n\t" \
-    "s_mov_b32 m0, %[ldst]\n\t" \
+    "s_add_u32 m0, %[ldst], 0x0\n\t" \
     "s_nop 0\n\t" \
     "global_load_lds_dwordx4 %[voff0], %[sbase]\n\t" \
     "v_mfma_scale_f32_32x32x64_f8f6f4 %[c1], v[250:255], v[238:243], %[c1], %[ws], %[sb1] op_sel:[0,1,0] op_sel_hi:[0,0,0] cbsz:2 blgp:2\n\t" \
@@ -341,7 +341,7 @@
     "global_load_lds_dwordx4 %[voff1], %[sbase]\n\t" \
     "v_mfma_scale_f32_32x32x64_f8f6f4 %[c2], v[250:255], v[244:249], %[c2], %[ws], %[sb2] op_sel:[0,1,0] op_sel_hi:[0,0,0] cbsz:2 blgp:2\n\t" \
     "ds_read_b128 %[a1h2], %[t2]\n\t" \
-    "ds_read_b128 %[w1], %[vbn] offset:4096\n\t" \
+    "ds_read_b128 %[w1], %[vb] offset:36864\n\t" \
     "s_mov_b32 m0, %[keep]\n\t"
 
 #define MX_SKIP0_ASM_Q2 \
@@ -360,9 +360,9 @@
     "ds_read_b128 v[244:247], %[xr2] offset:14336\n\t" \
     "ds_read_b64 v[248:249], %[yr2] offset:35840\n\t" \
     "v_mfma_f32_32x32x16_f16 %[c2], %[w0], %[a0h2], %[c2]\n\t" \
-    "ds_read_b128 v[250:253], %[vb] offset:8192\n\t" \
-    "ds_read_b64 v[254:255], %[vy]\n\t" \
-    "ds_read_b32 %[ws], %[vs]\n\t" \
+    "ds_read_b128 v[250:253], %[vb] offset:40960\n\t" \
+    "ds_read_b64 v[254:255], %[vy] offset:32768\n\t" \
+    "ds_read_b32 %[ws], %[vs] offset:32768\n\t" \
     "s_waitcnt vmcnt(2)\n\t" \
     "s_barrier\n\t" \
     "s_waitcnt lgkmcnt(9)\n\t" \
@@ -380,7 +380,7 @@
     "ds_read_b128 %[a0h1], %[t1]\n\t" \
     "v_mfma_f32_32x32x16_f16 %[c2], %[w1], %[a1h2], %[c2]\n\t" \
     "ds_read_b128 %[a0h2], %[t2]\n\t" \
-    "ds_read_b128 %[w0], %[vbn]\n\t" \
+    "ds_read_b128 %[w0], %[vb] offset:49152\n\t" \
     "s_waitcnt lgkmcnt(4)\n\t" \
     "s_cbranch_vccnz 1f\n\t" \
     "v_mfma_scale_f32_32x32x64_f8f6f4 %[c0], v[250:255], v[232:237], %[c0], %[ws], %[sb0] op_sel:[0,0,0] op_sel_hi:[0,1,0] cbsz:2 blgp:2\n\t" \
@@ -391,18 +391,18 @@
     "v_lshl_add_u32 %[t0], %[t0], 4, %[ab0]\n\t" \
     "v_lshl_add_u32 %[t1], %[t1], 4, %[ab1]\n\t" \
     "v_lshl_add_u32 %[t2], %[t2], 4, %[ab2]\n\t" \
-    "s_mov_b32 m0, %[ldst]\n\t" \
+    "s_add_u32 m0, %[ldst], 0x4000\n\t" \
     "s_nop 0\n\t" \
     "global_load_lds_dwordx4 %[voff0], %[sbase]\n\t" \
     "v_mfma_scale_f32_32x32x64_f8f6f4 %[c1], v[250:255], v[238:243], %[c1], %[ws], %[sb1] op_sel:[0,0,0] op_sel_hi:[0,1,0] cbsz:2 blgp:2\n\t" \
     "ds_read_b128 %[a1h0], %[t0]\n\t" \
     "ds_read_b128 %[a1h1], %[t1]\n\t" \
-    "s_add_u32 m0, %[ldst], 0x2000\n\t" \
+    "s_add_u32 m0, %[ldst], 0x6000\n\t" \
     "s_nop 0\n\t" \
     "global_load_lds_dwordx4 %[voff1], %[sbase]\n\t" \
     "v_mfma_scale_f32_32x32x64_f8f6f4 %[c2], v[250:255], v[244:249], %[c2], %[ws], %[sb2] op_sel:[0,0,0] op_sel_hi:[0,1,0] cbsz:2 blgp:2\n\t" \
     "ds_read_b128 %[a1h2], %[t2]\n\t" \
-    "ds_read_b128 %[w1], %[vbn] offset:4096\n\t" \
+    "ds_read_b128 %[w1], %[vb] offset:53248\n\t" \
     "s_mov_b32 m0, %[keep]\n\t"
 
 #define MX_SKIP0_ASM_Q3 \
@@ -421,9 +421,9 @@
     "ds_read_b128 v[244:247], %[xr2] offset:21504\n\t" \
     "ds_read_b64 v[248:249], %[yr2] offset:39424\n\t" \
     "v_mfma_f32_32x32x16_f16 %[c2], %[w0], %[a0h2], %[c2]\n\t" \
-    "ds_read_b128 v[250:253], %[vb] offset:8192\n\t" \
-    "ds_read_b64 v[254:255], %[vy]\n\t" \
-    "ds_read_b32 %[ws], %[vs]\n\t" \
+    "ds_read_b128 v[250:253], %[vb] offset:57344\n\t" \
+    "ds_read_b64 v[254:255], %[vy] offset:49152\n\t" \
+    "ds_read_b32 %[ws], %[vs] offset:49152\n\t" \
     "s_waitcnt vmcnt(2)\n\t" \
     "s_barrier\n\t" \
     "s_waitcnt lgkmcnt(9)\n\t" \
@@ -441,7 +441,7 @@
     "ds_read_b128 %[a0h1], %[t1]\n\t" \
     "v_mfma_f32_32x32x16_f16 %[c2], %[w1], %[a1h2], %[c2]\n\t" \
     "ds_read_b128 %[a0h2], %[t2]\n\t" \
-    "ds_read_b128 %[w0], %[vbn]\n\t" \
+    "ds_read_b128 %[w0], %[vb] offset:0\n\t" \
     "s_waitcnt lgkmcnt(4)\n\t" \
     "s_cbranch_vccnz 1f\n\t" \
     "v_mfma_scale_f32_32x32x64_f8f6f4 %[c0], v[250:255], v[232:237], %[c0], %[ws], %[sb0] op_sel:[0,1,0] op_sel_hi:[0,1,0] cbsz:2 blgp:2\n\t" \
@@ -452,18 +452,18 @@
     "v_lshl_add_u32 %[t0], %[t0], 4, %[nab0]\n\t" \
     "v_lshl_add_u32 %[t1], %[t1], 4, %[nab1]\n\t" \
     "v_lshl_add_u32 %[t2], %[t2], 4, %[nab2]\n\t" \
-    "s_mov_b32 m0, %[ldst]\n\t" \
+    "s_add_u32 m0, %[ldst], 0x8000\n\t" \
     "s_nop 0\n\t" \
     "global_load_lds_dwordx4 %[voff0], %[sbase]\n\t" \
     "v_mfma_scale_f32_32x32x64_f8f6f4 %[c1], v[250:255], v[238:243], %[c1], %[ws], %[sb1] op_sel:[0,1,0] op_sel_hi:[0,1,0] cbsz:2 blgp:2\n\t" \
     "ds_read_b128 %[a1h0], %[t0]\n\t" \
     "ds_read_b128 %[a1h1], %[t1]\n\t" \
-    "s_add_u32 m0, %[ldst], 0x2000\n\t" \
+    "s_add_u32 m0, %[ldst], 0xa000\n\t" \
     "s_nop 0\n\t" \
     "global_load_lds_dwordx4 %[voff1], %[sbase]\n\t" \
     "v_mfma_scale_f32_32x32x64_f8f6f4 %[c2], v[250:255], v[244:249], %[c2], %[ws], %[sb2] op_sel:[0,1,0] op_sel_hi:[0,1,0] cbsz:2 blgp:2\n\t" \
     "ds_read_b128 %[a1h2], %[t2]\n\t" \
-    "ds_read_b128 %[w1], %[vbn] offset:4096\n\t" \
+    "ds_read_b128 %[w1], %[vb] offset:4096\n\t" \
     "s_mov_b32 m0, %[keep]\n\t"
 
 #define MX_SLAB_ASM_Q3_LAST \
@@ -478,20 +478,20 @@
     "ds_read_b128 v[244:247], %[xr2] offset:21504\n\t" \
     "ds_read_b64 v[248:249], %[yr2] offset:39424\n\t" \
     "v_mfma_f32_32x32x16_f16 %[c2], %[w0], %[a0h2], %[c2]\n\t" \
-    "ds_read_b128 v[250:253], %[vb] offset:8192\n\t" \
-    "ds_read_b64 v[254:255], %[vy]\n\t" \
-    "ds_read_b32 %[ws], %[vs]\n\t" \
+    "ds_read_b128 v[250:253], %[vb] offset:57344\n\t" \
+    "ds_read_b64 v[254:255], %[vy] offset:49152\n\t" \
+    "ds_read_b32 %[ws], %[vs] offset:49152\n\t" \
     "s_waitcnt vmcnt(2) lgkmcnt(0)\n\t" \
     "s_barrier\n\t" \
     "v_mfma_f32_32x32x16_f16 %[c0], %[w1], %[a1h0], %[c0]\n\t" \
     "v_mfma_f32_32x32x16_f16 %[c1], %[w1], %[a1h1], %[c1]\n\t" \
     "v_mfma_f32_32x32x16_f16 %[c2], %[w1], %[a1h2], %[c2]\n\t" \
     "v_mfma_scale_f32_32x32x64_f8f6f4 %[c0], v[250:255], v[232:237], %[c0], %[ws], %[sb0] op_sel:[0,1,0] op_sel_hi:[0,1,0] cbsz:2 blgp:2\n\t" \
-    "s_mov_b32 m0, %[ldst]\n\t" \
+    "s_add_u32 m0, %[ldst], 0x8000\n\t" \
     "s_nop 0\n\t" \
     "global_load_lds_dwordx4 %[voff0], %[sbase]\n\t" \
     "v_mfma_scale_f32_32x32x64_f8f6f4 %[c1], v[250:255], v[238:243], %[c1], %[ws], %[sb1] op_sel:[0,1,0] op_sel_hi:[0,1,0] cbsz:2 blgp:2\n\t" \
-    "s_add_u32 m0, %[ldst], 0x2000\n\t" \
+    "s_add_u32 m0, %[ldst], 0xa000\n\t" \
     "s_nop 0\n\t" \
     "global_load_lds_dwordx4 %[voff1], %[sbase]\n\t" \
     "v_mfma_scale_f32_32x32x64_f8f6f4 %[c2], v[250:255], v[244:249], %[c2], %[ws], %[sb2] op_sel:[0,1,0] op_sel_hi:[0,1,0] cbsz:2 blgp:2\n\t" \
```
